# SamsungLabs/fcaf3d

Measured on AMD Instinct MI355X. Metric: scenes/sec fwd+bwd, ScanNet 100k-pt 2cm voxels, 1/2/4/8 MI355X, higher is better.
Workload: dtype f32

## Files before the change

### fcaf3d_amd/_lib.py

```python
import ctypes
import os
import re
import threading
import time

import torch

_HERE = os.path.dirname(os.path.abspath(__file__))
LIB_PATH = os.environ.get('FC_LIB') or os.path.join(_HERE, 'libfcaf3d_hip.so')
HEADER = os.path.join(os.path.dirname(_HERE), 'include', 'fcaf3d_hip.h')

_SCALARS = {'int': ctypes.c_int, 'int64_t': ctypes.c_int64, 'float': ctypes.c_float,
            'hipStream_t': ctypes.c_void_p}


def parse_header(path=HEADER):
    txt = open(path).read()
    txt = re.sub(r'/\*.*?\*/', '', txt, flags=re.S)
    protos = {}
    for m in re.finditer(r'\b(int64_t|int)\s+(fc_\w+)\s*\(([^)]*)\)\s*;', txt):
        ret, name, args = m.group(1), m.group(2), m.group(3)
        argl = []
        for a in args.split(','):
            a = ' '.join(a.split())
# ... 7 lines not shown
        protos[name] = (_SCALARS[ret], argl)
    return protos


EXEC_OPS = os.path.join(_HERE, 'csrc', 'exec_ops.h')


def parse_enums(path=EXEC_OPS):
    txt = re.sub(r'//[^\n]*', '', open(path).read())
    known, blocks = {}, []
    for m in re.finditer(r'\benum\s*\{([^}]*)\}', txt):
        block, nxt = {}, 0
        for item in filter(None, (s.strip() for s in m.group(1).split(','))):
            name, _, expr = (s.strip() for s in item.partition('='))
            if expr:
                nxt = sum(known[t] if t in known else int(t, 0) for t in (s.strip() for s in expr.split('+')))
            assert re.fullmatch(r'[A-Z]\w*', name) and name not in known, item
            block[name] = known[name] = nxt
            nxt += 1
        blocks.append(block)
    return blocks


ABI_VERSION = 10
_lib = None
_protos = None


def lib():
    global _lib, _protos
    if _lib is None:
        if not os.path.exists(LIB_PATH):
            raise RuntimeError(
                f'{LIB_PATH} is missing: build it with `python -m fcaf3d_amd.build` '
                '(hipcc --offload-arch=gfx950).  There is no CPU fallback.')
        l = ctypes.CDLL(LIB_PATH)
        _protos = parse_header()
        for name, (ret, args) in _protos.items():
            fn = getattr(l, name)
            fn.restype = ret
            fn.argtypes = [t for _, t in args]
        if l.fc_abi_version() != ABI_VERSION:
            raise RuntimeError(f'{LIB_PATH} speaks ABI version {l.fc_abi_version()}, this host code was written for {ABI_VERSION}: rebuild '
                               'with `python -m fcaf3d_amd.build`')
        _lib = l
    return _lib

# ... 107 lines not shown
```

### fcaf3d_amd/csrc/conv.hip

```cpp
#include "fc_common.h"
#include "../../include/fcaf3d_hip.h"
#ifdef FC_TRACE
__device__ unsigned long long* g_trace_buf_lds;
__device__ int g_trace_cap_lds;
extern "C" int fc_debug_trace_lds(unsigned long long* buf, int cap) {
  FC_HIP(hipMemcpyToSymbol(HIP_SYMBOL(g_trace_buf_lds), &buf, sizeof(buf)));
  FC_HIP(hipMemcpyToSymbol(HIP_SYMBOL(g_trace_cap_lds), &cap, sizeof(cap)));
  return FC_OK;
}
#define TR_BUF g_trace_buf_lds
#define TR_CAP g_trace_cap_lds
#endif
#include "fc_trace.h"

typedef float f32x16 __attribute__((ext_vector_type(16)));
typedef float f32x2 __attribute__((ext_vector_type(2)));
typedef float f32x4 __attribute__((ext_vector_type(4)));

__device__ __attribute__((aligned(16))) float g_zero_row[64];

__device__ int g_fc_prio;
extern "C" int fc_debug_set_prio(int mode) {
  FC_HIP(hipMemcpyToSymbol(HIP_SYMBOL(g_fc_prio), &mode, sizeof(mode)));
  return FC_OK;
// ... 1345 lines not shown
int fc_conv_fwd_pairs(const float* in, const float* W, const int* pair_in, const int* pair_cnt, const int* pair_pos,
                      float* out, int64_t n_in, int64_t n_out, int K, int Cin, int Cout, int flags, void* ws,
                      int64_t ws_bytes, hipStream_t stream) {
  return fc_conv_fwd_pairs_tiles(in, W, pair_in, pair_cnt, pair_pos, out, n_in, n_out, K, Cin, Cout, 0, flags, ws, ws_bytes, stream);
}

int64_t fc_x6_weight_image_bytes(int K, int R, int C) { return (int64_t)K * R * C * 6; }

int fc_x6_weight_image(const float* W, void* img, int K, int R, int C, int transposed, hipStream_t stream) {
  if (K < 1 || R < 32 || C < 64 || R % 32 != 0 || C % 64 != 0) return FC_EINVAL;
  const int64_t total = (int64_t)K * (R / 32) * (C / 64) * 256;
  const unsigned nb = (unsigned)fc_cdiv(total, 256);
  if (split_mode() == 2) {
    FC_HIP(hipMemsetAsync((char*)img + 4 * X6_IMG_AMAX_WORD, 0, FC_AMAX_SLOT_BYTES, stream));
    k_x6_weight_image<3><<<nb, 256, 0, stream>>>(W, (u32x4*)img, K, R, C, transposed);
    k_x6_weight_image<2><<<nb, 256, 0, stream>>>(W, (u32x4*)img, K, R, C, transposed);
  } else {
    k_x6_weight_image<0><<<nb, 256, 0, stream>>>(W, (u32x4*)img, K, R, C, transposed);
  }
  FC_CHECK_LAUNCH();
  return FC_OK;
}

int fc_x6_weight_images(const int64_t* desc, int n, int64_t total_blocks, hipStream_t stream) {
  if (!desc || n < 1 || total_blocks < 1 || total_blocks > 0x7fffffffll) return FC_EINVAL;
  const long long* d = reinterpret_cast<const long long*>(desc);
  if (split_mode() == 2) {
    k_x6_weight_images<4><<<(unsigned)fc_cdiv(n, 4), 256, 0, stream>>>(d, n);
    k_x6_weight_images<3><<<(unsigned)total_blocks, 256, 0, stream>>>(d, n);
    k_x6_weight_images<2><<<(unsigned)total_blocks, 256, 0, stream>>>(d, n);
  } else {
    k_x6_weight_images<0><<<(unsigned)total_blocks, 256, 0, stream>>>(d, n);
  }
  FC_CHECK_LAUNCH();
  return FC_OK;
}

}

template <int BMc, int BNc, bool HAS_NBR, int BKR, bool PAIRS>
__global__ __launch_bounds__(256, 2) void k_wgrad_mfma(const float* __restrict__ in, const float* __restrict__ gout,
                                                    const int* __restrict__ nbr, const int* __restrict__ row_index,
                                                    const int* __restrict__ cnt,
                                                    float* __restrict__ part, int64_t n_out, int K, int Cin, int Cout,
                                                    int64_t rows_per_split) {
  constexpr int TM = BMc / 64, TN = BNc / 64;
  constexpr int AR = BMc * BKR / 1024, GR = BNc * BKR / 1024;
  __shared__ __attribute__((aligned(16))) float As[BKR * BMc];
  __shared__ __attribute__((aligned(16))) float Gs[BKR * BNc];
  const int tid = threadIdx.x, lane = tid & 63, wave = tid >> 6;
  const int wr = wave >> 1, wc = wave & 1;
  const int r = lane & 31, h = lane >> 5;
  const int tiles_n = Cout / BNc, tiles_m = Cin / BMc;
  int y = blockIdx.y;
  const int tn = y % tiles_n; y /= tiles_n;
  const int tm = y % tiles_m; y /= tiles_m;
  const int k = y;
  const int ci0 = tm * BMc, co0 = tn * BNc;
  int64_t total = n_out;
// ... 566 lines not shown
```

### fcaf3d_amd/csrc/optim.hip

```cpp
#include "fc_common.h"

typedef float of4 __attribute__((ext_vector_type(4)));

#define SQ_BLOCKS 1024

__global__ __launch_bounds__(256) void k_sqsum_partial(const of4* __restrict__ g, int64_t n4, double* __restrict__ part) {
  __shared__ double red[4];
  double acc = 0.0;
  const int64_t stride = (int64_t)gridDim.x * 256;
  for (int64_t i = (int64_t)blockIdx.x * 256 + threadIdx.x; i < n4; i += 4 * stride) {
    of4 v[4];
#pragma unroll
    for (int u = 0; u < 4; ++u) {
      const int64_t j = i + u * stride;
      v[u] = j < n4 ? g[j] : of4{0.f, 0.f, 0.f, 0.f};
    }
#pragma unroll
    for (int u = 0; u < 4; ++u) {
      const float s = v[u][0] * v[u][0] + v[u][1] * v[u][1] + v[u][2] * v[u][2] + v[u][3] * v[u][3];
      acc += (double)s;
    }
  }
  for (int off = 32; off > 0; off >>= 1) acc += __shfl_xor(acc, off, 64);
  if ((threadIdx.x & 63) == 0) red[threadIdx.x >> 6] = acc;
  __syncthreads();
  if (threadIdx.x == 0) part[blockIdx.x] = (red[0] + red[1]) + (red[2] + red[3]);
}

__global__ __launch_bounds__(1024) void k_sqsum_final(const double* __restrict__ part, int nb, float max_norm,
                                                      float* __restrict__ out) {
  __shared__ double red[16];
  double acc = 0.0;
  for (int i = threadIdx.x; i < nb; i += 1024) acc += fc_ld(&part[i]);
  for (int off = 32; off > 0; off >>= 1) acc += __shfl_xor(acc, off, 64);
  if ((threadIdx.x & 63) == 0) red[threadIdx.x >> 6] = acc;
  __syncthreads();
  if (threadIdx.x == 0) {
    double t = 0.0;
    for (int w = 0; w < 16; ++w) t += red[w];
    const float norm = (float)sqrt(t);
    out[0] = norm;
    float c = 1.f;
    if (max_norm > 0.f) c = fminf(max_norm / (norm + 1e-6f), 1.f);
    out[1] = c;
  }
}

__global__ __launch_bounds__(256) void k_adamw(of4* __restrict__ p, const of4* __restrict__ g, of4* __restrict__ m,
                                               of4* __restrict__ v, int64_t n4, float lr, float b1, float b2, float eps,
                                               float wd, float step_size, float bc2_sqrt, const float* __restrict__ clip) {
  const int64_t i = (int64_t)blockIdx.x * 256 + threadIdx.x;
  if (i >= n4) return;
  const float c = clip ? fc_ld(&clip[1]) : 1.f;
  of4 pv = p[i], gv = g[i], mv = m[i], vv = v[i];
  const float decay = 1.f - lr * wd;
#pragma unroll
  for (int j = 0; j < 4; ++j) {
    const float gg = gv[j] * c;
    float pp = pv[j] * decay;
    const float mm = mv[j] + (gg - mv[j]) * (1.f - b1);
    const float v2 = vv[j] * b2 + (1.f - b2) * gg * gg;
    const float denom = sqrtf(v2) / bc2_sqrt + eps;
    pp -= step_size * (mm / denom);
    pv[j] = pp; mv[j] = mm; vv[j] = v2;
  }
  p[i] = pv; m[i] = mv; v[i] = vv;
}

extern "C" {

int64_t fc_grad_norm_ws_bytes(int64_t n) { return (int64_t)SQ_BLOCKS * (int64_t)sizeof(double); }

int fc_grad_norm(const float* g, int64_t n, float max_norm, float* out, void* ws, int64_t ws_bytes, hipStream_t stream) {
  if (n < 0 || n % 4 || !out) return FC_EINVAL;
  if (ws_bytes < fc_grad_norm_ws_bytes(n)) return FC_EWS;
  const int64_t n4 = n / 4;
  int nb = (int)fc_cdiv(n4 > 0 ? n4 : 1, 256 * 4);
  if (nb > SQ_BLOCKS) nb = SQ_BLOCKS;
  k_sqsum_partial<<<nb, 256, 0, stream>>>((const of4*)g, n4, (double*)ws);
  FC_CHECK_LAUNCH();
  k_sqsum_final<<<1, 1024, 0, stream>>>((const double*)ws, nb, max_norm, out);
  FC_CHECK_LAUNCH();
  return FC_OK;
}

int fc_adamw_step(float* p, const float* g, float* m, float* v, int64_t n, float lr, float beta1, float beta2, float eps,
                  float weight_decay, float bias_correction1, float bias_correction2, const float* norm_and_clip,
                  hipStream_t stream) {
  if (n < 0 || n % 4 || bias_correction1 <= 0.f || bias_correction2 <= 0.f) return FC_EINVAL;
  if (n == 0) return FC_OK;
  const int64_t n4 = n / 4;
  k_adamw<<<(unsigned)fc_cdiv(n4, 256), 256, 0, stream>>>((of4*)p, (const of4*)g, (of4*)m, (of4*)v, n4, lr, beta1, beta2, eps,
                                                         weight_decay, lr / bias_correction1, sqrtf(bias_correction2),
                                                         norm_and_clip);
  FC_CHECK_LAUNCH();
  return FC_OK;
}

}
```

### fcaf3d_amd/executor.py

```python
import os
import struct

import numpy as np
import torch

from . import _lib as L
from . import functional as Fn
from . import nn as MEnn

ENABLED = os.environ.get('FC_EXEC', '1') != '0'
PROBE = None
TRUSTED = None
KEEP_STATE = False


def _layouts():
    names, fields = {}, {}
    for block in L.parse_enums():
        names.update(block)
        *members, end = block
        op = names.get('OP_' + end[:-len('_END')]) if end.endswith('_END') else None
        if op is not None:
            fields[op] = {n[len(end) - 3:].lower().removesuffix('_p1'): (block[n], n.endswith('_P1')) for n in members}
    return {k: v for k, v in names.items() if k.startswith('OP_') or k in ('OPW', 'MAPW', 'ROW_OP', 'ROW_STREAM')}, fields


_NAMES, FIELDS = _layouts()
globals().update(_NAMES)


def word(op, field):
    return FIELDS[op][field][0]


ALIGN = 256
S_MAIN, S_HEAD, S_WGRAD = 0, 1, 2
EV_FORK, EV_HEAD_DONE, EV_W0, EV_W1, EV_WEND, EV_BWD0, EV_HB = 0, 8, 9, 10, 11, 12, 16


def _f(x):
    return struct.unpack('<q', struct.pack('<d', float(x)))[0]


def supported(det):
    bb, nh = det.backbone, det.neck_with_head
    if not (ENABLED and Fn.X6 and not (Fn.FLAGS & Fn.CONV_FMA) and Fn.STEM_COL and Fn.DGRAD_WT):
        return False
    if getattr(bb.BLOCK, 'expansion', 1) != 1 or det.spatial_sort:
        return False
    if 1 + nh.n_reg_outs + nh.n_classes > 64 or bb.conv1[0].in_channels != 3:
        return False
    return type(nh).forward_single is _FORWARD_SINGLE and type(nh).forward is _NECK_FORWARD


_FORWARD_SINGLE = _NECK_FORWARD = None


class NetProgram:
    def __init__(self, det, training, wgrad_async, head_overlap, tail0=False, keep_state=None):
        self.det = det
# ... 110 lines not shown
        self._amax_used += 1
        return i

    def amax_op(self, lst, stream, x, rows, cols):
        slot = self.amax_slot()
        self.emit(lst, OP_AMAX, stream, x=x, n=self.D(rows), c=cols, slot=slot)
        return slot

    def _build_weights(self):
        holder = self.det.__dict__.get('_exec_weights')
        if holder is None or holder.sig != self._sig:
            holder = self.det.__dict__['_exec_weights'] = _Weights(self.det, self.dev, self._sig)
        self.w = holder
        self.packed, self.gent_w, self.gents, self.images, self.ncol = holder.packed, holder.gent_w, holder.gents, holder.images, holder.ncol

    @property
    def weights_fresh(self):
        return self.w.fresh

    @weights_fresh.setter
    def weights_fresh(self, v):
        self.w.fresh = v

    def refresh_weights(self):
        self.w.refresh()

    def IMG(self, w, transposed):
        v = self.w.img_of[w.data_ptr()]
        assert v is not None and v[1 if transposed else 0] is not None, 'no split-bf16 image for this kernel shape'
        return self.S(v[1 if transposed else 0])

    def _build(self):
        det = self.det
        bb, nh = det.backbone, det.neck_with_head
        tr = self.training
        F, Bk = self.ops_f, self.ops_b
        tape = []
        self.relu_outs = []
        self.small = []
        relu, elu, none = Fn.ACT['relu'], Fn.ACT['elu'], Fn.ACT['none']
        grad = {}
        head_grads = {}
        self._pready = {}
        small_rows = []
        flushed = [0]

        head_lvl = [None]
        head_written = {}

        def wrote(*params):
            for prm in params:
                self._pready[id(prm)] = len(Bk)
            if head_lvl[0] is not None:
                head_written.setdefault(head_lvl[0], []).extend(params)

        def flush_small(stream):
            n = len(small_rows) - flushed[0]
            if n:
                self.emit(Bk, OP_SMALL_GRADS, stream, desc=self.DY('small_desc'), first=2 * flushed[0], count=2 * n)
                for _, _, _, w_, b_ in small_rows[flushed[0]:]:
                    wrote(w_, b_)
                flushed[0] = len(small_rows)
        head_wgrads = [0]

        def head_wfin(stream):
            lo = 1 if self.tail0 else 0
            self.emit(Bk, OP_HEAD_WFIN, stream, part=self.SA(head_part[lo].data_ptr()), nl=self.nl - lo, r=Cn, ld=64, n_reg=n_reg, n_cls=n_cls,
                      g_cent=self.G(nh.centerness_conv.kernel), g_reg=self.G(nh.reg_conv.kernel), g_cls=self.G(nh.cls_conv.kernel),
                      bias_part=self.SA(bias_part[lo].data_ptr()), g_bias=self.G(nh.cls_conv.bias))
# ... 33 lines not shown
                return grad[t], (grad2.pop(t)[0] if t in grad2 else None)
            if t in grad2:
                flush2(t)
            return grad[t]

        def got(t):
            if t in grad2:
                flush2(t)
            return grad[t]

        def emit_wgrad(cur, **fields):
            if self.wgrad_async:
                ev = EV_W0 if cur == S_MAIN else EV_W1
                self.emit(Bk, OP_RECORD, cur, event=ev)
                self.emit(Bk, OP_WAIT, S_WGRAD, event=ev)
            self.emit(Bk, OP_WGRAD, wstream(cur), **fields)

        AMAX = Fn.X6 and Fn.split_mode() == 2
        amax_f = {}
        amax_of = {}
        if AMAX:
            self.amax_slot()
            self.emit(F, OP_CLEAR, S_MAIN, dst=self.SA(self._amax_buf.data_ptr()), bytes=0)

        def fwd_amax(x, rows, cols, stream):
            if not AMAX:
                return -1
            if x in amax_of:
                return amax_of[x]
            if (x, stream) not in amax_f:
                amax_f[(x, stream)] = self.amax_op(F, stream, x, rows, cols)
            return amax_f[(x, stream)]

        producer = {}
        grad_src = {}

        def conv(x, mod, mname, rows_in, rows_out, stream=S_MAIN):
            Cin, Cout = mod.in_channels, mod.out_channels
            y = self.T(rows_out, Cout)
            m = self.M(mname)
            ax = fwd_amax(x, rows_in, Cin, stream)
            self.emit(F, OP_CONV, stream, x=x, img=self.IMG(mod.kernel, False), map=m, dir=0, out=y, n=-1, cin=Cin, cout=Cout, amax_x=ax)
            producer[y] = (len(F) - 1, rows_out, Cout)
            if tr:
                def bwd():
                    gy = take(y, rows_out, Cout) if stream == S_MAIN else got(y)
                    gx = self.T(rows_in, Cin, 'b')
                    ag = (amax_of[gy] if gy in amax_of else self.amax_op(Bk, stream, gy, rows_out, Cout)) if AMAX else -1
                    self.emit(Bk, OP_CONV, stream, x=gy, img=self.IMG(mod.kernel, True), map=m, dir=1, out=gx, n=-1, cin=Cout, cout=Cin, amax_x=ag)
                    grad_src[gx] = (len(Bk) - 1, rows_in, Cin, stream)
                    emit_wgrad(stream, x=x, gout=gy, map=m, gw=self.G(mod.kernel), n=-1, cin=Cin, cout=Cout, amax_x=ax, amax_gout=ag)
                    wrote(mod.kernel)
                    accumulate(x, gx, rows_in, Cin, stream)
                tape.append((stream, bwd))
            return y

        def gemm(x, w_tensor, rows, Cin, Cout, gw_dst, stream=S_MAIN):
            y = self.T(rows, Cout)
            ax = fwd_amax(x, rows, Cin, stream)
            self.emit(F, OP_CONV, stream, x=x, img=self.IMG(w_tensor, False), map=-1, dir=0, out=y, n=self.D(rows), cin=Cin, cout=Cout, amax_x=ax)
            producer[y] = (len(F) - 1, rows, Cout)
            if tr:
                def bwd():
                    gy = take(y, rows, Cout) if stream == S_MAIN else got(y)
                    gx = self.T(rows, Cin, 'b')
                    ag = (amax_of[gy] if gy in amax_of else self.amax_op(Bk, stream, gy, rows, Cout)) if AMAX else -1
                    self.emit(Bk, OP_CONV, stream, x=gy, img=self.IMG(w_tensor, True), map=-1, dir=1, out=gx, n=self.D(rows), cin=Cout, cout=Cin, amax_x=ag)
                    grad_src[gx] = (len(Bk) - 1, rows, Cin, stream)
                    emit_wgrad(stream, x=x, gout=gy, map=-1, gw=gw_dst, n=self.D(rows), cin=Cin, cout=Cout, amax_x=ax, amax_gout=ag)
                    if w_tensor is self.packed:
                        head_wgrads[0] += 1
                        if head_wgrads[0] == self.nl - (1 if self.tail0 else 0) and self.wgrad_async:
                            head_wfin(S_WGRAD)
                    accumulate(x, gx, rows, Cin, stream)
                tape.append((stream, bwd))
            return y

        def bn(x, mod, act, rows, res=None, stream=S_MAIN, add=None):
            assert add is None or res is None
            b = mod.bn
            C = b.num_features
            y = self.T(rows, C)
            mean, var, cnt = (self.T('one', C), self.T('one', C), self.T('one', 1)) if tr else (-1, -1, -1)
# ... 167 lines not shown
            outs = [self.AL(cent_all, off, 1), self.AL(bbox_all, off, n_reg), self.AL(cls_all, off, n_cls), self.AL(cmax_all, off, 1)]
            self.emit(F, OP_HEAD_FWD, hs, y=y, ld=64, bias=self.S(nh.cls_conv.bias), scale=self.S(nh.scales[i].scale), n=self.D(x_rows), n_reg=n_reg,
                      n_cls=n_cls, cent=outs[0], bbox=outs[1], cls=outs[2], cmax=outs[3])
            if tr:
                def bwd_head(y=y, outs=outs, off=off, hs=hs, rows=x_rows, lvl=i):
                    gy = self.T(rows, 64, 'b')
                    gin = [self.AL(g, off, c) for g, c in zip(self.gout_idx, (1, n_reg, n_cls))]
                    agy = -1
                    if AMAX:
                        agy = amax_of[gy] = self.amax_slot()
                    self.emit(Bk, OP_HEAD_BWD, hs, y=y, ld=64, scale=self.S(nh.scales[lvl].scale), bbox=outs[1], g_cent=gin[0], g_bbox=gin[1],
                              g_cls=gin[2], n=self.D(rows), n_reg=n_reg, n_cls=n_cls, gy=gy, gs_row=-1, g_scale=self.G(nh.scales[lvl].scale),
                              bias_part=self.SA(bias_part[lvl].data_ptr()), amax_gy=agy)
                    wrote(nh.scales[lvl].scale)
                    grad[y] = gy
                tape.append((hs, bwd_head))
                if hs == S_HEAD:
                    tape.append((S_HEAD, ('join', x, x_rows, x_C, i)))
        if self.head_overlap:
            self.emit(F, OP_RECORD, S_HEAD, event=EV_HEAD_DONE)
            self.emit(F, OP_WAIT, S_MAIN, event=EV_HEAD_DONE)
        if AMAX:
            n_fwd_slots = self._amax_used
            self.patch(F[0], bytes=self.AMAX_SLOT_BYTES * n_fwd_slots)
            if tr:
                self.emit(Bk, OP_CLEAR, S_MAIN, dst=self.SA(self._amax_buf.data_ptr() + self.AMAX_SLOT_BYTES * n_fwd_slots), bytes=0)
                clear_b = len(Bk) - 1
        if tr:
            if self.head_overlap:
                self.emit(Bk, OP_RECORD, S_MAIN, event=EV_BWD0)
                self.emit(Bk, OP_WAIT, S_HEAD, event=EV_BWD0)
                branches, cur_b = [], None
                for s, e in reversed(tape):
                    if s != S_HEAD:
                        continue
                    if isinstance(e, tuple):
                        cur_b = [e, []]
                        branches.append(cur_b)
                    else:
                        cur_b[1].append(e)
                for (_, xt, rows, C, lvl), ems in sorted(branches, key=lambda b: b[0][4]):
                    saved = grad.pop(xt, None)
                    assert saved is None
                    head_lvl[0] = lvl
                    for e in ems:
                        e()
                    flush_small(S_HEAD)
# ... 146 lines not shown
                    if self._need[i] > wsb[i]:
                        self._ws[i] = torch.empty(int(self._need[i] * 5 // 4) + (1 << 20), dtype=torch.uint8, device=self.dev)
                continue
            if rc != 0:
                raise RuntimeError(f'fc_exec failed: {"invalid argument" if rc == -1 else "hipError %d" % rc}')
            return

    def decisions(self, st):
        assert self.keep_state, 'this program does not store the stem\'s normalised output: build it under executor.KEEP_STATE'
        fa, addr, dims = st['fa'], st['addr'], st['dims']

        def view(idx, rows, C, dtype):
            n = int(dims[self.dim_names[rows]])
            o = int(addr[idx] - fa.data_ptr())
            return fa[o:o + n * C * 4].view(dtype).view(n, C)
        relu = [(view(t, r, C, torch.float32) > 0).cpu() for t, r, C in self.relu_outs]
        return relu, view(*self.pool_arg, torch.int32).cpu()

    def forward(self, st):
        trusted = (TRUSTED is not None and TRUSTED.w is self.w) or (not self.training and getattr(self.det, 'static_weights', False))
        if not (self.weights_fresh and trusted):
            self.refresh_weights()
        ev = self.images.event
        if ev is not None:
            torch.cuda.current_stream().wait_event(ev)
        if self.training:
            return _NetFn.apply(self._anchor, self, st)
        return self._forward(st)

    def _forward(self, st):
        dims = st['dims']
        fa = torch.empty(self._arena_bytes(dims, 'f'), dtype=torch.uint8, device=self.dev)
        addr = self.addr0.copy()
        base = (fa.data_ptr() + ALIGN - 1) // ALIGN * ALIGN
        self._fill_arena(addr, dims, 'f', base)
        addr[self.dyn['x0']] = st['x'].F.data_ptr()
        addr[self.dyn['seg1']] = st['seg1'].data_ptr()
        for k, t in st['dyn'].items():
            addr[self.dyn[k]] = t.data_ptr()
        ai, ap, ad, ab = self._al
        fwd_alias = addr[ap] != 0
        addr[ai[fwd_alias]] = addr[ap[fwd_alias]] + dims[ad[fwd_alias]] * ab[fwd_alias]
        st['fa'], st['addr'] = fa, addr
        self._run(self.ops_f, addr, st)
        n = st['n_all']
        nh = self.det.neck_with_head
        outs = []
# ... 102 lines not shown


class _Weights:

    def __init__(self, det, dev, sig):
        nh = det.neck_with_head
        self.det, self.sig = det, sig
        head = (nh.centerness_conv, nh.reg_conv, nh.cls_conv)
        convs = [m for m in det.modules() if isinstance(m, MEnn.MinkowskiConvolution) and m not in head]
        self.gents = [m for m in det.modules() if isinstance(m, MEnn.MinkowskiGenerativeConvolutionTranspose)]
        C = nh.centerness_conv.in_channels
        self.ncol = 1 + nh.n_reg_outs + nh.n_classes
        self.packed = torch.zeros((1, C, 64), dtype=torch.float32, device=dev)
        self.gent_w = [torch.empty((1, m.in_channels, 8 * m.out_channels), dtype=torch.float32, device=dev) for m in self.gents]
        ws = [m.kernel for m in convs] + [self.packed] + self.gent_w
        self.images = Fn.WeightImages(ws)
        self.img_of = {}
        for w in ws:
            K = 1 if w.dim() == 2 else w.shape[0]
            self.img_of[w.data_ptr()] = self.images.table.get((w.data_ptr(), K, w.shape[-2], w.shape[-1]))
        self.fresh = False

    @torch.no_grad()
    def refresh(self):
        nh = self.det.neck_with_head
        torch.cat((nh.centerness_conv.kernel, nh.reg_conv.kernel, nh.cls_conv.kernel), dim=1, out=self.packed[0][:, :self.ncol])
        for m, w in zip(self.gents, self.gent_w):
            w.view(m.in_channels, 8, m.out_channels).copy_(m.kernel.permute(1, 0, 2))
        self.images.build()
        self.fresh = True


class _NetFn(torch.autograd.Function):

    @staticmethod
    def forward(ctx, anchor, prog, st):
        ctx.prog, ctx.st = prog, st
        outs = prog._forward(st)
        ctx.mark_non_differentiable(outs[3])
        return outs

    @staticmethod
    def backward(ctx, g_cent, g_bbox, g_cls, _g_max, g_x0=None):
        ctx.prog._backward(ctx.st, g_cent, g_bbox, g_cls, g_x0)
        return None, None, None


def program_for(det, training, tail0=False):
    if not supported(det):
        return None
    nh = det.neck_with_head
    if tail0 and min(det.backbone.n_outs, 4) < 2:
        return None
    key = (bool(training), bool(Fn.WGRAD_ASYNC), bool(nh.head_overlap), bool(tail0))
    keep = bool(KEEP_STATE)
    fuse = bool(Fn.BN_FUSE)
    mode = Fn.split_mode() if Fn.X6 else -1
    cache = det.__dict__.setdefault('_programs', {})
    sig = NetProgram.signature(det)
    prog = cache.get(key + (fuse, mode, keep))
    if prog is None or prog._sig != sig:
        prog = cache[key + (fuse, mode, keep)] = NetProgram(det, *key, keep_state=keep)
    if getattr(prog.w, 'split_mode', mode) != mode:
        prog.w.fresh = False
    prog.w.split_mode = mode
    return prog
```

### fcaf3d_amd/functional.py

```python
import os

import torch

from . import _lib as L

CONV_FMA = 1 << 0
CONV_BM_SHIFT, CONV_BN_SHIFT, CONV_TILE_MASK = 4, 6, 3
CONV_S_SHIFT, CONV_S_MASK = 8, 255
CONV_WGRAD_PIPE_OFF = 1 << 16
CONV_PIPE_OFF = 1 << 17
CONV_PIPE_ON = 1 << 18
CONV_WGRAD_DEEP = 1 << 19
CONV_WGRAD_PIPE_ON = 1 << 20
CONV_GLDS = 1 << 21
CONV_GLDS_OFF = 1 << 22
CONV_WT = 1 << 23
CONV_SPLIT = 1 << 24
CONV_IMAGE = 1 << 26
CONV_FLAT = 1 << 27
CONV_WGRAD_MULTI_OFF = 1 << 29
CONV_WGRAD_MULTI_FIRST = 1 << 30

FLAGS = int(os.environ.get('FC_FLAGS', '0'), 0)

# ... 544 lines not shown

class WeightImages:

    def __init__(self, weights):
        ents, off = [], 0
        self.table = {}
        dev = None
        for w in weights:
            if w.dim() == 2:
                K, (Cin, Cout) = 1, w.shape
            else:
                K, Cin, Cout = w.shape
            dev = w.device
            pair = [None, None]
            for tr, (R, C) in ((0, (Cin, Cout)), (1, (Cout, Cin))):
                if R % 32 or C % 64 or not w.is_contiguous():
                    continue
                nbytes = L.query('fc_x6_weight_image_bytes', K, R, C)
                pair[tr] = (off, nbytes, K, R, C)
                off += (nbytes + 255) // 256 * 256
            if pair[0] or pair[1]:
                ents.append((w, pair))
        self.n = 0
        if not ents:
            return
        self.buf = torch.empty(off, dtype=torch.uint8, device=dev)
        desc, blk = [], 0
        for w, pair in ents:
            views = []
            for tr in (0, 1):
                if pair[tr] is None:
                    views.append(None)
                    continue
                o, nb, K, R, C = pair[tr]
                v = self.buf[o:o + nb]
                views.append(v)
                desc += [w.data_ptr(), v.data_ptr(), K, R, C, tr, blk, views[0].data_ptr() if (tr == 1 and views[0] is not None) else 0]
                blk += K * (R // 32) * (C // 64)
            K = 1 if w.dim() == 2 else w.shape[0]
            self.table[(w.data_ptr(), K, w.shape[-2], w.shape[-1])] = tuple(views)
        self.n = len(desc) // 8
        self.blocks = blk
        self.desc = torch.tensor(desc, dtype=torch.int64).to(dev)
        self.event = None

    def build(self):
        if self.n:
            L.call('fc_x6_weight_images', L.ptr(self.desc), self.n, self.blocks, L.stream())
            self.event = torch.cuda.Event()
            self.event.record()
```

### fcaf3d_amd/runner.py

```python
import os

import torch

from . import _lib as L
from . import dist as D
from .flat import FlatParams


class FlatAdamW:

    def __init__(self, flat, lr=1e-3, betas=(0.9, 0.999), eps=1e-8, weight_decay=1e-2):
        self.flat = flat
        self.defaults = dict(lr=lr, betas=tuple(betas), eps=eps, weight_decay=weight_decay, amsgrad=False)
        self.param_groups = [dict(self.defaults, params=flat.params)]
        self.exp_avg = torch.zeros_like(flat.data)
        self.exp_avg_sq = torch.zeros_like(flat.data)
        self.norm_clip = torch.zeros(2, dtype=torch.float32, device=flat.data.device)
        self.steps = 0

    def zero_grad(self, set_to_none=True):
        for p in self.flat.params:
            p.grad = None
        self.flat.complete = False

    def step(self, max_norm=None, gathered=False):
        f = self.flat
        if not f.data.is_cuda:
            raise RuntimeError('FlatAdamW runs on the GPU only (HIP); CPU parameters take torch.optim.AdamW')
        if not gathered and not getattr(f, 'complete', False):
            f.gather()
        g = self.param_groups[0]
        self.steps += 1
        b1, b2 = g['betas']
        clip = None
        if max_norm is not None:
            ws = L.workspace(L.query('fc_grad_norm_ws_bytes', f.n), f.data.device)
            L.call('fc_grad_norm', L.ptr(f.grad), f.n, float(max_norm), L.ptr(self.norm_clip), L.ptr(ws), ws.numel(), L.stream())
            clip = self.norm_clip
        L.call('fc_adamw_step', L.ptr(f.data), L.ptr(f.grad), L.ptr(self.exp_avg), L.ptr(self.exp_avg_sq), f.n, float(g['lr']),
               float(b1), float(b2), float(g['eps']), float(g['weight_decay']), 1.0 - b1 ** self.steps, 1.0 - b2 ** self.steps,
               L.ptr(clip), L.stream())
        return self.norm_clip[0].clone() if clip is not None else None

    def _views(self, buf):
        return [buf[o:o + p.numel()].view(p.shape) for p, o in zip(self.flat.params, self.flat.offsets)]

    def state_dict(self):
        m, v = self._views(self.exp_avg), self._views(self.exp_avg_sq)
        state = {i: dict(step=torch.tensor(float(self.steps)), exp_avg=m[i].clone(), exp_avg_sq=v[i].clone())
                 for i in range(len(m))} if self.steps else {}
        group = {k: val for k, val in self.param_groups[0].items() if k != 'params'}
        group['params'] = list(range(len(self.flat.params)))
        return dict(state=state, param_groups=[group])

    def load_state_dict(self, sd):
        m, v = self._views(self.exp_avg), self._views(self.exp_avg_sq)
        steps = 0
        with torch.no_grad():
            self.exp_avg.zero_()
            self.exp_avg_sq.zero_()
            for i, st in sd['state'].items():
                m[int(i)].copy_(st['exp_avg'])
                v[int(i)].copy_(st['exp_avg_sq'])
                steps = int(st['step'])
# ... 99 lines not shown
        self.flat = FlatParams(self.params) if use_flat else None
        self.optimizer = build_optimizer(model, optimizer_cfg, flat=self.flat)
        self.lr = build_lr_updater(self.optimizer, lr_config) if lr_config else None
        self.averager = D.GradientAverager(self.params, bucket_mb=bucket_mb, flat=self.flat)
        self.last_grad_norm = None
        self.phase_s = [0.0, 0.0, 0.0, 0.0]
        from . import functional as Fn
        self.images = None
        if self.flat is not None and Fn.X6:
            from .nn import MinkowskiConvolution
            ws = [m.kernel for m in model.modules() if isinstance(m, MinkowskiConvolution) and m.kernel.requires_grad]
            self.images = Fn.WeightImages(ws)
            self._image_ws, self.images_version = ws, None

    @classmethod
    def from_config(cls, model, cfg, **kw):
        return cls(model, cfg.optimizer, cfg.get('optimizer_config'), cfg.get('lr_config'), **kw)

    def invalidate_images(self):
        for pr in getattr(self.model, '_programs', {}).values():
            pr.weights_fresh = False
        self.images_version = None

    def _build_images(self, side_stream):
        from . import functional as Fn
        if side_stream:
            side, main = Fn.wgrad_stream(self.flat.data.device), torch.cuda.current_stream()
            side.wait_stream(main)
            with torch.cuda.stream(side):
                self.images.build()
        else:
            self.images.build()
        self.images_version = sum(w._version for w in self._image_ws)

    def _program(self):
        from . import executor
        if self.flat is None or not hasattr(self.model, 'backbone') or not self.model.training:
            return None
        return executor.program_for(self.model, True)

    def __call__(self, batch, next_batch=None):
        from . import functional as Fn
        import time
        ph = self.phase_s
        t0 = time.perf_counter()
        self._bound_run_ahead()
        if next_batch is not None and hasattr(self.model, 'prefetch'):
            self.model.prefetch(next_batch['points'], gt=True)
        t1 = time.perf_counter()
        ph[0] += t1 - t0
        self.optimizer.zero_grad(set_to_none=True)
        Fn._flat_pass_done()
        prog = self._program()
        if prog is not None:
            ver = sum(w._version for w in self._image_ws) if self.images is not None else None
            if not prog.weights_fresh or getattr(self, '_prog_version', None) != ver:
                prog.refresh_weights()
                self._prog_version = ver
        elif self.images is not None and self.images.n:
            if self.images_version != sum(w._version for w in self._image_ws):
                self._build_images(side_stream=False)
            Fn.PREBUILT, Fn.PREBUILT_EVENT = self.images.table, self.images.event
        from . import executor
        executor.TRUSTED = prog
        try:
            losses = self.model(return_loss=True, **batch)
            loss = parse_losses(losses)
            t2 = time.perf_counter()
            ph[1] += t2 - t1
            loss.backward()
            t3 = time.perf_counter()
            ph[2] += t3 - t2
        finally:
            Fn.PREBUILT, Fn.PREBUILT_EVENT = {}, None
            executor.TRUSTED = None
        self.averager.finish()
        if isinstance(self.optimizer, FlatAdamW):
            self.last_grad_norm = self.optimizer.step(self.max_norm, gathered=bool(self.averager.buckets))
            for pr in getattr(self.model, '_programs', {}).values():
                pr.weights_fresh = False
            if prog is not None:
                side, main = Fn.wgrad_stream(self.flat.data.device), torch.cuda.current_stream()
                side.wait_stream(main)
                with torch.cuda.stream(side):
                    prog.refresh_weights()
                self.images_version = None
            elif self.images is not None and self.images.n:
                self._build_images(side_stream=True)
            ph[3] += time.perf_counter() - t3
            return loss, losses
        if self.max_norm is not None:
            self.last_grad_norm = torch.nn.utils.clip_grad_norm_(self.params, self.max_norm, norm_type=self.norm_type)
        self.optimizer.step()
        return loss, losses

    def _bound_run_ahead(self, depth=int(os.environ.get('FC_RUN_AHEAD', '2'))):
        if not self.params or not self.params[0].is_cuda:
            return
        evs = self.__dict__.setdefault('_step_events', [])
        if len(evs) >= depth:
            e0 = evs.pop(0)
            if not e0.query():
                import time
                t0 = time.perf_counter()
                e0.synchronize()
                L.HOST_WAIT[0] += time.perf_counter() - t0
        e = torch.cuda.Event()
        e.record()
        evs.append(e)

    def epoch_end(self):
# ... 12 lines not shown
```

### include/fcaf3d_hip.h

```cpp
#ifndef FCAF3D_HIP_H
#define FCAF3D_HIP_H
#include <stdint.h>

#ifndef __HIP_PLATFORM_AMD__
typedef struct ihipStream_t* hipStream_t;
#endif

#ifdef __cplusplus
extern "C" {
#endif

#define FC_ABI_VERSION 10
#ifndef FC_AMAX_SLOT_BYTES
#define FC_AMAX_SLOT_BYTES 2048
#endif
int fc_abi_version(void);


int fc_voxelize(const float* points, int64_t n, int pt_stride, int batch_idx, float voxel_size, float feat_div,
                int nfeat, int* coords, float* feats, hipStream_t stream);

int fc_augment_voxelize(const float* points, int64_t n_src, int pt_stride, const int* sample_idx, int64_t n_out,
                        const float* xform_host, int batch_idx, float voxel_size, float feat_div, int nfeat, int* coords,
                        float* feats, float* points_out, hipStream_t stream);

int fc_morton_keys(const int* coords, int64_t n, long long* keys, hipStream_t stream);

int fc_scan_flags(const unsigned char* flags, int64_t n, int* pos, int* total_dev, void* ws, int64_t ws_bytes,
                  hipStream_t stream);
int fc_compact_rows(const unsigned char* flags, const int* pos, int64_t n, int* kept, int64_t m, hipStream_t stream);

int64_t fc_hash_unique_ws_bytes(int64_t n);
int fc_hash_unique(const int* coords, int64_t n, int q, unsigned long long* table_keys, int* table_vals, int64_t cap,
                   int* out_coords, int* first_idx, int* inverse, int* n_out_dev, void* ws, int64_t ws_bytes,
                   hipStream_t stream);
// ... 40 lines not shown
#define FC_CONV_FMA (1 << 0)
#define FC_CONV_BM_SHIFT 4
#define FC_CONV_BN_SHIFT 6
#define FC_CONV_TILE_MASK 3
#define FC_CONV_S_SHIFT 8
#define FC_CONV_S_MASK 255
#define FC_CONV_WGRAD_PIPE_OFF (1 << 16)
#define FC_CONV_PIPE_OFF (1 << 17)
#define FC_CONV_PIPE_ON (1 << 18)
#define FC_CONV_WGRAD_DEEP (1 << 19)
#define FC_CONV_WGRAD_PIPE_ON (1 << 20)
#define FC_CONV_GLDS (1 << 21)
#define FC_CONV_GLDS_OFF (1 << 22)
#define FC_CONV_WT (1 << 23)
#define FC_CONV_SPLIT (1 << 24)
#define FC_CONV_IMAGE (1 << 26)
#define FC_CONV_FLAT (1 << 27)
#define FC_CONV_WGRAD_MULTI_OFF (1 << 29)
#define FC_CONV_WGRAD_MULTI_FIRST (1 << 30)

int64_t fc_x6_weight_image_bytes(int K, int R, int C);
int fc_x6_weight_image(const float* W, void* img, int K, int R, int C, int transposed, hipStream_t stream);
int fc_x6_weight_images(const int64_t* desc, int n, int64_t total_blocks, hipStream_t stream);

int64_t fc_conv_fwd_ws_bytes(int64_t n_out, int K, int Cin, int Cout, int flags);
int fc_conv_fwd(const float* in, const float* W, const int* nbr, const int* out_index, float* out, int64_t n_in,
                int64_t n_out, int K, int Cin, int Cout, int flags, void* ws, int64_t ws_bytes, hipStream_t stream);

int64_t fc_conv_fwd_pairs_ws_bytes(int64_t n_out, int K, int Cout);
int fc_conv_fwd_pairs(const float* in, const float* W, const int* pair_in, const int* pair_cnt, const int* pair_pos,
                      float* out, int64_t n_in, int64_t n_out, int K, int Cin, int Cout, int flags, void* ws,
                      int64_t ws_bytes, hipStream_t stream);

int fc_conv_fwd_pairs_tiles(const float* in, const float* W, const int* pair_in, const int* pair_cnt, const int* pair_pos,
                            float* out, int64_t n_in, int64_t n_out, int K, int Cin, int Cout, int64_t live_tiles, int flags,
                            void* ws, int64_t ws_bytes, hipStream_t stream);

int64_t fc_conv_stats_blocks(int64_t n_out, int K, int Cin, int Cout, int flags, int pairs);
int fc_conv_fwd_stats(const float* in, const float* W, const int* nbr, const int* out_index, float* out, int64_t n_in,
                      int64_t n_out, int K, int Cin, int Cout, int flags, void* ws, int64_t ws_bytes, float* stats,
                      hipStream_t stream);
int fc_conv_fwd_pairs_tiles_stats(const float* in, const float* W, const int* pair_in, const int* pair_cnt, const int* pair_pos,
                                  float* out, int64_t n_in, int64_t n_out, int K, int Cin, int Cout, int64_t live_tiles, int flags,
                                  void* ws, int64_t ws_bytes, float* stats, hipStream_t stream);
int fc_conv_fwd_bn_bwd_stats(const float* in, const float* W, const int* nbr, const int* out_index, float* out, int64_t n_in,
                             int64_t n_out, int K, int Cin, int Cout, int flags, void* ws, int64_t ws_bytes, float* stats,
// ... 150 lines not shown
int64_t fc_nms_bev_ws_bytes(int nseg, int stride);
int fc_nms_bev(const float* boxes, const int* counts_dev, int nseg, int stride, float thresh, int rotated,
               unsigned long long* mask_ws, int64_t ws_bytes, int* keep, int* keep_count, hipStream_t stream);
int fc_boxes_iou_bev(const float* boxes_a, int n, const float* boxes_b, int m, int rotated, float* out,
                     hipStream_t stream);


#define FC_MERGE_TO_BOTTOM 1
#define FC_MERGE_WITH_YAW 2
#define FC_MERGE_XF_FLIP_H (1ull << 32)
#define FC_MERGE_XF_FLIP_V (1ull << 33)
int64_t fc_merge_sorted_segments_ws_bytes(int nseg_out, int max_total);
int fc_merge_sorted_segments(const int64_t* desc, int nseg_out, int K, const int* counts_dev, const int* keep, int keep_stride,
                             const int64_t* ord, int ord_stride, const float* scores, int score_stride, const float* boxes,
                             int flags, int max_total, int cap, float* out_boxes, float* out_scores, int* out_src,
                             int* out_count, int stride_out, void* ws, int64_t ws_bytes, hipStream_t stream);


int64_t fc_grad_norm_ws_bytes(int64_t n);
int fc_grad_norm(const float* g, int64_t n, float max_norm, float* out, void* ws, int64_t ws_bytes, hipStream_t stream);
int fc_adamw_step(float* p, const float* g, float* m, float* v, int64_t n, float lr, float beta1, float beta2, float eps,
                  float weight_decay, float bias_correction1, float bias_correction2, const float* norm_and_clip,
                  hipStream_t stream);

int fc_set_bf16_fast(int on);

int fc_set_split_mode(int mode);
int fc_get_split_mode(void);
int fc_amax(const float* x, int64_t n, unsigned* slot, hipStream_t stream);
int fc_conv_amax_hint(const unsigned* amax_in, const unsigned* amax_gout);
int fc_amax_out_hint(unsigned* amax_word);
int fc_debug_set_h3r(int mode);


int fc_exec_op_words(void);
int64_t fc_exec_probe_read(float* ms, int64_t* meta, int64_t cap);
int fc_exec_map_words(void);
int fc_exec(const int64_t* ops, int64_t op_begin, int64_t op_end, const int64_t* addr, const int64_t* dims, const int64_t* maps,
            const int64_t* streams, const int64_t* ws, const int64_t* ws_bytes, int64_t* ws_need, const int64_t* cfg);

#ifdef __cplusplus
}
#endif
#endif
```

Before: 512.3.

## Fuse weight-image amax into AdamW step and defer image wait to first conv

```diff
diff --git a/fcaf3d_amd/_lib.py b/fcaf3d_amd/_lib.py
--- a/fcaf3d_amd/_lib.py
+++ b/fcaf3d_amd/_lib.py
@@ -53,7 +53,7 @@
     return blocks
 
 
-ABI_VERSION = 10
+ABI_VERSION = 11
 _lib = None
 _protos = None
 
diff --git a/fcaf3d_amd/csrc/conv.hip b/fcaf3d_amd/csrc/conv.hip
--- a/fcaf3d_amd/csrc/conv.hip
+++ b/fcaf3d_amd/csrc/conv.hip
@@ -1391,19 +1391,25 @@
   return FC_OK;
 }
 
-int fc_x6_weight_images(const int64_t* desc, int n, int64_t total_blocks, hipStream_t stream) {
-  if (!desc || n < 1 || total_blocks < 1 || total_blocks > 0x7fffffffll) return FC_EINVAL;
+int fc_x6_weight_images_phases(const int64_t* desc, int n, int64_t total_blocks, int phases, hipStream_t stream) {
+  if (!desc || n < 1 || total_blocks < 1 || total_blocks > 0x7fffffffll || phases < 1 || phases > 7) return FC_EINVAL;
   const long long* d = reinterpret_cast<const long long*>(desc);
   if (split_mode() == 2) {
-    k_x6_weight_images<4><<<(unsigned)fc_cdiv(n, 4), 256, 0, stream>>>(d, n);
-    k_x6_weight_images<3><<<(unsigned)total_blocks, 256, 0, stream>>>(d, n);
-    k_x6_weight_images<2><<<(unsigned)total_blocks, 256, 0, stream>>>(d, n);
-  } else {
+    if (phases & 1) k_x6_weight_images<4><<<(unsigned)fc_cdiv(n, 4), 256, 0, stream>>>(d, n);
+    if (phases & 2) k_x6_weight_images<3><<<(unsigned)total_blocks, 256, 0, stream>>>(d, n);
+    if (phases & 4) k_x6_weight_images<2><<<(unsigned)total_blocks, 256, 0, stream>>>(d, n);
+  } else if (phases & 4) {
     k_x6_weight_images<0><<<(unsigned)total_blocks, 256, 0, stream>>>(d, n);
   }
   FC_CHECK_LAUNCH();
   return FC_OK;
 }
+
+int fc_x6_weight_images(const int64_t* desc, int n, int64_t total_blocks, hipStream_t stream) {
+  return fc_x6_weight_images_phases(desc, n, total_blocks, 7, stream);
+}
+
+int64_t fc_x6_weight_image_amax_offset(void) { return 4 * (int64_t)X6_IMG_AMAX_WORD; }
 
 }
 
diff --git a/fcaf3d_amd/csrc/optim.hip b/fcaf3d_amd/csrc/optim.hip
--- a/fcaf3d_amd/csrc/optim.hip
+++ b/fcaf3d_amd/csrc/optim.hip
@@ -46,6 +46,17 @@
   }
 }
 
+__device__ __forceinline__ void adamw_elem(float& p, float g, float& m, float& v, float c, float decay, float omb1, float b2, float omb2,
+                                           float eps, float step_size, float bc2_sqrt) {
+#pragma clang fp contract(off)
+  const float gg = g * c;
+  const float mm = __builtin_fmaf(omb1, __builtin_fmaf(c, g, -m), m);
+  const float v2 = __builtin_fmaf(b2, v, gg * (omb2 * gg));
+  const float denom = sqrtf(v2) / bc2_sqrt + eps;
+  p = __builtin_fmaf(decay, p, -(step_size * (mm / denom)));
+  m = mm; v = v2;
+}
+
 __global__ __launch_bounds__(256) void k_adamw(of4* __restrict__ p, const of4* __restrict__ g, of4* __restrict__ m,
                                                of4* __restrict__ v, int64_t n4, float lr, float b1, float b2, float eps,
                                                float wd, float step_size, float bc2_sqrt, const float* __restrict__ clip) {
@@ -53,18 +64,87 @@
   if (i >= n4) return;
   const float c = clip ? fc_ld(&clip[1]) : 1.f;
   of4 pv = p[i], gv = g[i], mv = m[i], vv = v[i];
-  const float decay = 1.f - lr * wd;
+  const float decay = __builtin_fmaf(-lr, wd, 1.f), omb1 = 1.f - b1, omb2 = 1.f - b2;
 #pragma unroll
   for (int j = 0; j < 4; ++j) {
-    const float gg = gv[j] * c;
-    float pp = pv[j] * decay;
-    const float mm = mv[j] + (gg - mv[j]) * (1.f - b1);
-    const float v2 = vv[j] * b2 + (1.f - b2) * gg * gg;
-    const float denom = sqrtf(v2) / bc2_sqrt + eps;
-    pp -= step_size * (mm / denom);
-    pv[j] = pp; mv[j] = mm; vv[j] = v2;
+    float pj = pv[j], mj = mv[j], vj = vv[j];
+    adamw_elem(pj, gv[j], mj, vj, c, decay, omb1, b2, omb2, eps, step_size, bc2_sqrt);
+    pv[j] = pj; mv[j] = mj; vv[j] = vj;
   }
   p[i] = pv; m[i] = mv; v[i] = vv;
+}
+
+__device__ __forceinline__ int seg_last_le(const long long* __restrict__ seg, int nseg, long long x) {
+  int lo = -1, hi = nseg - 1;
+  while (lo < hi) {
+    const int mid = (lo + hi + 1) >> 1;
+    if (seg[3 * mid] <= x) lo = mid; else hi = mid - 1;
+  }
+  return lo;
+}
+__device__ __forceinline__ void seg_fold(unsigned m, long long slot) {
+  unsigned* w = reinterpret_cast<unsigned*>(slot) + (blockIdx.x & (FC_AMAX_SUB - 1)) * FC_AMAX_STRIDE;
+  if (m > __hip_atomic_load(w, __ATOMIC_RELAXED, __HIP_MEMORY_SCOPE_AGENT)) atomicMax(w, m);
+}
+
+__global__ __launch_bounds__(256) void k_adamw_amax(of4* __restrict__ p, const of4* __restrict__ g, of4* __restrict__ m,
+                                                    of4* __restrict__ v, int64_t n4, float lr, float b1, float b2, float eps,
+                                                    float wd, float step_size, float bc2_sqrt, const float* __restrict__ clip,
+                                                    const long long* __restrict__ seg, int nseg) {
+  const int64_t i = (int64_t)blockIdx.x * 256 + threadIdx.x;
+  const bool live = i < n4;
+  const int64_t il = live ? i : n4 - 1;
+  const float c = clip ? fc_ld(&clip[1]) : 1.f;
+  of4 pv = p[il], gv = g[il], mv = m[il], vv = v[il];
+  const int wave = __builtin_amdgcn_readfirstlane((int)(threadIdx.x >> 6));
+  const long long b0 = (long long)blockIdx.x * 1024, x0 = b0 + wave * 256;
+  const int rb = seg_last_le(seg, nseg, b0);
+  const bool block_in = rb >= 0 && seg[3 * rb + 1] >= b0 + 1024;
+  const int r = block_in ? rb : seg_last_le(seg, nseg, x0);
+  const long long rend = r >= 0 ? seg[3 * r + 1] : 0;
+  const float decay = __builtin_fmaf(-lr, wd, 1.f), omb1 = 1.f - b1, omb2 = 1.f - b2;
+#pragma unroll
+  for (int j = 0; j < 4; ++j) {
+    float pj = pv[j], mj = mv[j], vj = vv[j];
+    adamw_elem(pj, gv[j], mj, vj, c, decay, omb1, b2, omb2, eps, step_size, bc2_sqrt);
+    pv[j] = pj; mv[j] = mj; vv[j] = vj;
+  }
+  unsigned am = 0u;
+  if (live) {
+    p[i] = pv; m[i] = mv; v[i] = vv;
+#pragma unroll
+    for (int j = 0; j < 4; ++j) {
+      const unsigned u = __float_as_uint(pv[j]) & 0x7fffffffu;
+      am = (u > am && u < 0x7f800000u) ? u : am;
+    }
+  }
+  const int lane = threadIdx.x & 63;
+  if (rend >= x0 + 256) {
+#pragma unroll
+    for (int off = 32; off > 0; off >>= 1) { const unsigned o = (unsigned)__shfl_xor((int)am, off, 64); am = o > am ? o : am; }
+    if (block_in) {
+      __shared__ unsigned red[4];
+      if (lane == 0) red[wave] = am;
+      __syncthreads();
+      if (threadIdx.x == 0) {
+        unsigned t = red[0];
+#pragma unroll
+        for (int k = 1; k < 4; ++k) t = red[k] > t ? red[k] : t;
+        seg_fold(t, seg[3 * r + 2]);
+      }
+    } else if (lane == 0) {
+      seg_fold(am, seg[3 * r + 2]);
+    }
+    return;
+  }
+  const bool next_in = r + 1 < nseg && seg[3 * (r + 1)] < x0 + 256;
+  if (rend <= x0 && !next_in) return;
+#pragma unroll
+  for (int off = 8; off > 0; off >>= 1) { const unsigned o = (unsigned)__shfl_xor((int)am, off, 64); am = o > am ? o : am; }
+  const long long xg = x0 + (lane >> 4) * 64;
+  int q = r;
+  while (q + 1 < nseg && seg[3 * (q + 1)] <= xg) ++q;
+  if (q >= 0 && (lane & 15) == 0 && seg[3 * q + 1] > xg) seg_fold(am, seg[3 * q + 2]);
 }
 
 extern "C" {
@@ -97,4 +177,19 @@
   return FC_OK;
 }
 
+int fc_adamw_step_amax(float* p, const float* g, float* m, float* v, int64_t n, float lr, float beta1, float beta2, float eps,
+                       float weight_decay, float bias_correction1, float bias_correction2, const float* norm_and_clip,
+                       const int64_t* seg, int nseg, hipStream_t stream) {
+  if (nseg < 0 || (nseg > 0 && !seg)) return FC_EINVAL;
+  if (nseg == 0) return fc_adamw_step(p, g, m, v, n, lr, beta1, beta2, eps, weight_decay, bias_correction1, bias_correction2, norm_and_clip, stream);
+  if (n < 0 || n % 4 || bias_correction1 <= 0.f || bias_correction2 <= 0.f) return FC_EINVAL;
+  if (n == 0) return FC_OK;
+  const int64_t n4 = n / 4;
+  k_adamw_amax<<<(unsigned)fc_cdiv(n4, 256), 256, 0, stream>>>((of4*)p, (const of4*)g, (of4*)m, (of4*)v, n4, lr, beta1, beta2, eps,
+                                                              weight_decay, lr / bias_correction1, sqrtf(bias_correction2),
+                                                              norm_and_clip, reinterpret_cast<const long long*>(seg), nseg);
+  FC_CHECK_LAUNCH();
+  return FC_OK;
 }
+
+}
diff --git a/fcaf3d_amd/executor.py b/fcaf3d_amd/executor.py
--- a/fcaf3d_amd/executor.py
+++ b/fcaf3d_amd/executor.py
@@ -35,7 +35,8 @@
 
 ALIGN = 256
 S_MAIN, S_HEAD, S_WGRAD = 0, 1, 2
-EV_FORK, EV_HEAD_DONE, EV_W0, EV_W1, EV_WEND, EV_BWD0, EV_HB = 0, 8, 9, 10, 11, 12, 16
+EV_FORK, EV_HEAD_DONE, EV_W0, EV_W1, EV_WEND, EV_BWD0, EV_IMG, EV_HB = 0, 8, 9, 10, 11, 12, 13, 16
+DEFER_IMAGE_WAIT = True
 
 
 def _f(x):
@@ -192,8 +193,8 @@
     def weights_fresh(self, v):
         self.w.fresh = v
 
-    def refresh_weights(self):
-        self.w.refresh()
+    def refresh_weights(self, phases=7):
+        self.w.refresh(phases)
 
     def IMG(self, w, transposed):
         v = self.w.img_of[w.data_ptr()]
@@ -215,6 +216,17 @@
         small_rows = []
         flushed = [0]
 
+        self.defer_wait = bool(tr and self.wgrad_async and DEFER_IMAGE_WAIT)
+        self.image_idx = set()
+        img_waited = [not self.defer_wait]
+        if self.defer_wait:
+            self.emit(F, OP_RECORD, S_WGRAD, event=EV_IMG)
+
+        def image_wait():
+            if not img_waited[0]:
+                self.emit(F, OP_WAIT, S_MAIN, event=EV_IMG)
+                img_waited[0] = True
+
         head_lvl = [None]
         head_written = {}
 
@@ -294,6 +306,7 @@
         if AMAX:
             self.amax_slot()
             self.emit(F, OP_CLEAR, S_MAIN, dst=self.SA(self._amax_buf.data_ptr()), bytes=0)
+            clear_f = len(F) - 1
 
         def fwd_amax(x, rows, cols, stream):
             if not AMAX:
@@ -312,7 +325,10 @@
             y = self.T(rows_out, Cout)
             m = self.M(mname)
             ax = fwd_amax(x, rows_in, Cin, stream)
+            assert img_waited[0] or stream == S_MAIN
+            image_wait()
             self.emit(F, OP_CONV, stream, x=x, img=self.IMG(mod.kernel, False), map=m, dir=0, out=y, n=-1, cin=Cin, cout=Cout, amax_x=ax)
+            self.image_idx.add(int(F[-1][word(OP_CONV, 'img')]))
             producer[y] = (len(F) - 1, rows_out, Cout)
             if tr:
                 def bwd():
@@ -330,7 +346,10 @@
         def gemm(x, w_tensor, rows, Cin, Cout, gw_dst, stream=S_MAIN):
             y = self.T(rows, Cout)
             ax = fwd_amax(x, rows, Cin, stream)
+            assert img_waited[0] or stream == S_MAIN
+            image_wait()
             self.emit(F, OP_CONV, stream, x=x, img=self.IMG(w_tensor, False), map=-1, dir=0, out=y, n=self.D(rows), cin=Cin, cout=Cout, amax_x=ax)
+            self.image_idx.add(int(F[-1][word(OP_CONV, 'img')]))
             producer[y] = (len(F) - 1, rows, Cout)
             if tr:
                 def bwd():
@@ -544,7 +563,7 @@
             self.emit(F, OP_WAIT, S_MAIN, event=EV_HEAD_DONE)
         if AMAX:
             n_fwd_slots = self._amax_used
-            self.patch(F[0], bytes=self.AMAX_SLOT_BYTES * n_fwd_slots)
+            self.patch(F[clear_f], bytes=self.AMAX_SLOT_BYTES * n_fwd_slots)
             if tr:
                 self.emit(Bk, OP_CLEAR, S_MAIN, dst=self.SA(self._amax_buf.data_ptr() + self.AMAX_SLOT_BYTES * n_fwd_slots), bytes=0)
                 clear_b = len(Bk) - 1
@@ -737,7 +756,7 @@
         if not (self.weights_fresh and trusted):
             self.refresh_weights()
         ev = self.images.event
-        if ev is not None:
+        if ev is not None and not (self.defer_wait and self.images.stream in (L.stream(), Fn.wgrad_stream(self.dev).cuda_stream)):
             torch.cuda.current_stream().wait_event(ev)
         if self.training:
             return _NetFn.apply(self._anchor, self, st)
@@ -886,13 +905,19 @@
         self.fresh = False
 
     @torch.no_grad()
-    def refresh(self):
+    def refresh(self, phases=7):
         nh = self.det.neck_with_head
         torch.cat((nh.centerness_conv.kernel, nh.reg_conv.kernel, nh.cls_conv.kernel), dim=1, out=self.packed[0][:, :self.ncol])
         for m, w in zip(self.gents, self.gent_w):
             w.view(m.in_channels, 8, m.out_channels).copy_(m.kernel.permute(1, 0, 2))
-        self.images.build()
+        self.images.build(phases)
         self.fresh = True
+
+    def seg_sources(self):
+        nh = self.det.neck_with_head
+        src = {self.packed.data_ptr(): [nh.centerness_conv.kernel, nh.reg_conv.kernel, nh.cls_conv.kernel]}
+        src.update({w.data_ptr(): [m.kernel] for m, w in zip(self.gents, self.gent_w)})
+        return src
 
 
 class _NetFn(torch.autograd.Function):
@@ -917,14 +942,15 @@
     if tail0 and min(det.backbone.n_outs, 4) < 2:
         return None
     key = (bool(training), bool(Fn.WGRAD_ASYNC), bool(nh.head_overlap), bool(tail0))
+    defer = bool(DEFER_IMAGE_WAIT)
     keep = bool(KEEP_STATE)
     fuse = bool(Fn.BN_FUSE)
     mode = Fn.split_mode() if Fn.X6 else -1
     cache = det.__dict__.setdefault('_programs', {})
     sig = NetProgram.signature(det)
-    prog = cache.get(key + (fuse, mode, keep))
+    prog = cache.get(key + (fuse, mode, keep, defer))
     if prog is None or prog._sig != sig:
-        prog = cache[key + (fuse, mode, keep)] = NetProgram(det, *key, keep_state=keep)
+        prog = cache[key + (fuse, mode, keep, defer)] = NetProgram(det, *key, keep_state=keep)
     if getattr(prog.w, 'split_mode', mode) != mode:
         prog.w.fresh = False
     prog.w.split_mode = mode
diff --git a/fcaf3d_amd/functional.py b/fcaf3d_amd/functional.py
--- a/fcaf3d_amd/functional.py
+++ b/fcaf3d_amd/functional.py
@@ -590,6 +590,7 @@
             if pair[0] or pair[1]:
                 ents.append((w, pair))
         self.n = 0
+        self.owners = []
         if not ents:
             return
         self.buf = torch.empty(off, dtype=torch.uint8, device=dev)
@@ -607,13 +608,41 @@
                 blk += K * (R // 32) * (C // 64)
             K = 1 if w.dim() == 2 else w.shape[0]
             self.table[(w.data_ptr(), K, w.shape[-2], w.shape[-1])] = tuple(views)
+            self.owners.append((w, views[0] if views[0] is not None else views[1]))
         self.n = len(desc) // 8
         self.blocks = blk
         self.desc = torch.tensor(desc, dtype=torch.int64).to(dev)
         self.event = None
-
-    def build(self):
+        self.stream = None
+
+    ZERO, AMAX, IMAGE = 1, 2, 4
+
+    def build(self, phases=7):
         if self.n:
-            L.call('fc_x6_weight_images', L.ptr(self.desc), self.n, self.blocks, L.stream())
+            L.call('fc_x6_weight_images_phases', L.ptr(self.desc), self.n, self.blocks, int(phases), L.stream())
             self.event = torch.cuda.Event()
             self.event.record()
+            self.stream = L.stream()
+
+    def zero_slots(self):
+        if self.n:
+            L.call('fc_x6_weight_images_phases', L.ptr(self.desc), self.n, self.blocks, self.ZERO, L.stream())
+
+    def seg_table(self, flat, sources=None):
+        from .flat import ALIGN
+        if not self.n:
+            return None
+        slot_off = L.query('fc_x6_weight_image_amax_offset')
+        base, rows = flat.data.data_ptr(), []
+        for w, owner in self.owners:
+            for src in (sources or {}).get(w.data_ptr(), [w]):
+                f = getattr(src, '_fc_flat', None)
+                if f is None or f[0] is not flat or src.data_ptr() != base + 4 * f[1]:
+                    return None
+                first, end = f[1], f[1] + -(-src.numel() // ALIGN) * ALIGN
+                assert first % ALIGN == 0 and end <= flat.n, 'slices of the flat buffers are 256-byte aligned'
+                rows.append((first, end, owner.data_ptr() + slot_off))
+        rows.sort()
+        for a, b in zip(rows, rows[1:]):
+            assert a[1] <= b[0], 'two image entries share weights'
+        return torch.tensor(rows, dtype=torch.int64).to(flat.data.device), len(rows)
diff --git a/fcaf3d_amd/runner.py b/fcaf3d_amd/runner.py
--- a/fcaf3d_amd/runner.py
+++ b/fcaf3d_amd/runner.py
@@ -5,6 +5,9 @@
 from . import _lib as L
 from . import dist as D
 from .flat import FlatParams
+
+
+AMAX_FROM_ADAMW = True
 
 
 class FlatAdamW:
@@ -23,7 +26,7 @@
             p.grad = None
         self.flat.complete = False
 
-    def step(self, max_norm=None, gathered=False):
+    def step(self, max_norm=None, gathered=False, seg=None):
         f = self.flat
         if not f.data.is_cuda:
             raise RuntimeError('FlatAdamW runs on the GPU only (HIP); CPU parameters take torch.optim.AdamW')
@@ -37,9 +40,13 @@
             ws = L.workspace(L.query('fc_grad_norm_ws_bytes', f.n), f.data.device)
             L.call('fc_grad_norm', L.ptr(f.grad), f.n, float(max_norm), L.ptr(self.norm_clip), L.ptr(ws), ws.numel(), L.stream())
             clip = self.norm_clip
-        L.call('fc_adamw_step', L.ptr(f.data), L.ptr(f.grad), L.ptr(self.exp_avg), L.ptr(self.exp_avg_sq), f.n, float(g['lr']),
-               float(b1), float(b2), float(g['eps']), float(g['weight_decay']), 1.0 - b1 ** self.steps, 1.0 - b2 ** self.steps,
-               L.ptr(clip), L.stream())
+        scalars = (f.n, float(g['lr']), float(b1), float(b2), float(g['eps']), float(g['weight_decay']), 1.0 - b1 ** self.steps,
+                   1.0 - b2 ** self.steps, L.ptr(clip))
+        if seg is not None:
+            L.call('fc_adamw_step_amax', L.ptr(f.data), L.ptr(f.grad), L.ptr(self.exp_avg), L.ptr(self.exp_avg_sq), *scalars,
+                   L.ptr(seg[0]), seg[1], L.stream())
+        else:
+            L.call('fc_adamw_step', L.ptr(f.data), L.ptr(f.grad), L.ptr(self.exp_avg), L.ptr(self.exp_avg_sq), *scalars, L.stream())
         return self.norm_clip[0].clone() if clip is not None else None
 
     def _views(self, buf):
@@ -185,16 +192,29 @@
             pr.weights_fresh = False
         self.images_version = None
 
-    def _build_images(self, side_stream):
+    def _build_images(self, side_stream, phases=7):
         from . import functional as Fn
         if side_stream:
             side, main = Fn.wgrad_stream(self.flat.data.device), torch.cuda.current_stream()
             side.wait_stream(main)
             with torch.cuda.stream(side):
-                self.images.build()
+                self.images.build(phases)
         else:
-            self.images.build()
+            self.images.build(phases)
         self.images_version = sum(w._version for w in self._image_ws)
+
+    def _amax_seg(self, prog):
+        from . import functional as Fn
+        imgs = prog.w.images if prog is not None else self.images
+        if not (AMAX_FROM_ADAMW and Fn.X6 and Fn.split_mode() == 2 and imgs is not None and imgs.n):
+            return None, None
+        cache = self.__dict__.setdefault('_seg_cache', {})
+        key = id(imgs)
+        if key not in cache or cache[key][0] is not imgs:
+            cache.clear()
+            cache[key] = (imgs, imgs.seg_table(self.flat, prog.w.seg_sources() if prog is not None else None))
+        seg = cache[key][1]
+        return (imgs, seg) if seg is not None else (None, None)
 
     def _program(self):
         from . import executor
@@ -239,17 +259,21 @@
             executor.TRUSTED = None
         self.averager.finish()
         if isinstance(self.optimizer, FlatAdamW):
-            self.last_grad_norm = self.optimizer.step(self.max_norm, gathered=bool(self.averager.buckets))
+            imgs, seg = self._amax_seg(prog)
+            if seg is not None:
+                imgs.zero_slots()
+            phases = 7 if seg is None else imgs.IMAGE
+            self.last_grad_norm = self.optimizer.step(self.max_norm, gathered=bool(self.averager.buckets), seg=seg)
             for pr in getattr(self.model, '_programs', {}).values():
                 pr.weights_fresh = False
             if prog is not None:
                 side, main = Fn.wgrad_stream(self.flat.data.device), torch.cuda.current_stream()
                 side.wait_stream(main)
                 with torch.cuda.stream(side):
-                    prog.refresh_weights()
+                    prog.refresh_weights(phases)
                 self.images_version = None
             elif self.images is not None and self.images.n:
-                self._build_images(side_stream=True)
+                self._build_images(side_stream=True, phases=phases)
             ph[3] += time.perf_counter() - t3
             return loss, losses
         if self.max_norm is not None:
diff --git a/include/fcaf3d_hip.h b/include/fcaf3d_hip.h
--- a/include/fcaf3d_hip.h
+++ b/include/fcaf3d_hip.h
@@ -10,7 +10,7 @@
 extern "C" {
 #endif
 
-#define FC_ABI_VERSION 10
+#define FC_ABI_VERSION 11
 #ifndef FC_AMAX_SLOT_BYTES
 #define FC_AMAX_SLOT_BYTES 2048
 #endif
@@ -97,6 +97,8 @@
 int64_t fc_x6_weight_image_bytes(int K, int R, int C);
 int fc_x6_weight_image(const float* W, void* img, int K, int R, int C, int transposed, hipStream_t stream);
 int fc_x6_weight_images(const int64_t* desc, int n, int64_t total_blocks, hipStream_t stream);
+int fc_x6_weight_images_phases(const int64_t* desc, int n, int64_t total_blocks, int phases, hipStream_t stream);
+int64_t fc_x6_weight_image_amax_offset(void);
 
 int64_t fc_conv_fwd_ws_bytes(int64_t n_out, int K, int Cin, int Cout, int flags);
 int fc_conv_fwd(const float* in, const float* W, const int* nbr, const int* out_index, float* out, int64_t n_in,
@@ -293,6 +295,9 @@
 int fc_adamw_step(float* p, const float* g, float* m, float* v, int64_t n, float lr, float beta1, float beta2, float eps,
                   float weight_decay, float bias_correction1, float bias_correction2, const float* norm_and_clip,
                   hipStream_t stream);
+int fc_adamw_step_amax(float* p, const float* g, float* m, float* v, int64_t n, float lr, float beta1, float beta2, float eps,
+                       float weight_decay, float bias_correction1, float bias_correction2, const float* norm_and_clip,
+                       const int64_t* seg, int nseg, hipStream_t stream);
 
 int fc_set_bf16_fast(int on);
 
```

Result: no change. 516.9, median of 6 (+0.9%).
